# liwanyue123/SRBD-NMPC-Solver

Measured on AMD Instinct MI355X. Metric: SRBD OCP-QP solves/sec (N=20, nx=12, nu=12, fp64) at 1/2/4/8 MI355X, higher is better.
Workload: dtype f64

## Files before the change

srbd-nmpc-solver_amd/csrc/qp_group.h:

```cpp
#pragma once

#include <hip/hip_runtime.h>

#include <type_traits>
#include <utility>

namespace srbd {

constexpr int kMaxDim = 12;
constexpr int kGroup = 16;
constexpr int kVecLane = 15;

template <int I>
using ic = std::integral_constant<int, I>;

template <int B, int E, typename F>
__device__ __forceinline__ void sfor(F&& f) {
  if constexpr (B < E) {
    f(ic<B>{});
    sfor<B + 1, E>(static_cast<F&&>(f));
  }
}
template <int B, int E, typename F>
__device__ __forceinline__ void sfor_down(F&& f) {
  if constexpr (B < E) {
    f(ic<E - 1>{});
    sfor_down<B, E - 1>(static_cast<F&&>(f));
  }
}

template <int SRC>
__device__ __forceinline__ double bc(double v) {
  static_assert(SRC >= 0 && SRC < kGroup, "row_newbcast source lane");
  return __builtin_amdgcn_update_dpp(0.0, v, 0x150 + SRC, 0xf, 0xf, true);
}

template <int SRC>
__device__ __forceinline__ float bc(float v) {
  static_assert(SRC >= 0 && SRC < kGroup, "row_newbcast source lane");
  return __builtin_bit_cast(
      float, __builtin_amdgcn_update_dpp(0, __builtin_bit_cast(int, v), 0x150 + SRC, 0xf, 0xf, true));
}

__device__ __forceinline__ void lds_wave_fence() {
  asm volatile("" ::: "memory");
  __builtin_amdgcn_wave_barrier();
}

template <typename T>
__device__ __forceinline__ void opaque(T& x) {
  asm volatile("" : "+v"(x));
}
template <typename T, int... Is>
__device__ __forceinline__ void launder_impl(T (&v)[12], std::integer_sequence<int, Is...>) {
  (opaque(v[Is]), ...);
}
template <typename T>
__device__ __forceinline__ void launder(T (&v)[12]) {
  launder_impl(v, std::make_integer_sequence<int, 12>{});
}

#define SRBD_FMAC_DPP(D, S0, S1, LANE) "v_fmac_f64_dpp " D ", " S0 ", " S1 " row_newbcast:" #LANE " row_mask:0xf bank_mask:0xf\n\t"

template <int SRC>
__device__ __forceinline__ void fma_bcast_src(double (&C)[12], const double (&X)[12], double y) {
  static_assert(SRC >= 0 && SRC < kGroup, "row_newbcast source lane");
  asm volatile(
      "s_nop 1\n\t"
      "v_fmac_f64_dpp %0, %12, %24 row_newbcast:%25 row_mask:0xf bank_mask:0xf\n\t"
      "v_fmac_f64_dpp %1, %13, %24 row_newbcast:%25 row_mask:0xf bank_mask:0xf\n\t"
      "v_fmac_f64_dpp %2, %14, %24 row_newbcast:%25 row_mask:0xf bank_mask:0xf\n\t"
      "v_fmac_f64_dpp %3, %15, %24 row_newbcast:%25 row_mask:0xf bank_mask:0xf\n\t"
      "v_fmac_f64_dpp %4, %16, %24 row_newbcast:%25 row_mask:0xf bank_mask:0xf\n\t"
      "v_fmac_f64_dpp %5, %17, %24 row_newbcast:%25 row_mask:0xf bank_mask:0xf\n\t"
      "v_fmac_f64_dpp %6, %18, %24 row_newbcast:%25 row_mask:0xf bank_mask:0xf\n\t"
      "v_fmac_f64_dpp %7, %19, %24 row_newbcast:%25 row_mask:0xf bank_mask:0xf\n\t"
      "v_fmac_f64_dpp %8, %20, %24 row_newbcast:%25 row_mask:0xf bank_mask:0xf\n\t"
      "v_fmac_f64_dpp %9, %21, %24 row_newbcast:%25 row_mask:0xf bank_mask:0xf\n\t"
      "v_fmac_f64_dpp %10, %22, %24 row_newbcast:%25 row_mask:0xf bank_mask:0xf\n\t"
      "v_fmac_f64_dpp %11, %23, %24 row_newbcast:%25 row_mask:0xf bank_mask:0xf"
      : "+v"(C[0]), "+v"(C[1]), "+v"(C[2]), "+v"(C[3]), "+v"(C[4]), "+v"(C[5]), "+v"(C[6]),
        "+v"(C[7]), "+v"(C[8]), "+v"(C[9]), "+v"(C[10]), "+v"(C[11])
      : "v"(X[0]), "v"(X[1]), "v"(X[2]), "v"(X[3]), "v"(X[4]), "v"(X[5]), "v"(X[6]), "v"(X[7]),
        "v"(X[8]), "v"(X[9]), "v"(X[10]), "v"(X[11]), "v"(y), "i"(SRC));
}

__device__ __forceinline__ void fma_bcast_lanes(double (&C)[12], double x, double y) {
  asm volatile(
      "s_nop 1\n\t"
      "v_fmac_f64_dpp %0, %12, %13 row_newbcast:0 row_mask:0xf bank_mask:0xf\n\t"
      "v_fmac_f64_dpp %1, %12, %13 row_newbcast:1 row_mask:0xf bank_mask:0xf\n\t"
      "v_fmac_f64_dpp %2, %12, %13 row_newbcast:2 row_mask:0xf bank_mask:0xf\n\t"
      "v_fmac_f64_dpp %3, %12, %13 row_newbcast:3 row_mask:0xf bank_mask:0xf\n\t"
      "v_fmac_f64_dpp %4, %12, %13 row_newbcast:4 row_mask:0xf bank_mask:0xf\n\t"
      "v_fmac_f64_dpp %5, %12, %13 row_newbcast:5 row_mask:0xf bank_mask:0xf\n\t"
      "v_fmac_f64_dpp %6, %12, %13 row_newbcast:6 row_mask:0xf bank_mask:0xf\n\t"
      "v_fmac_f64_dpp %7, %12, %13 row_newbcast:7 row_mask:0xf bank_mask:0xf\n\t"
      "v_fmac_f64_dpp %8, %12, %13 row_newbcast:8 row_mask:0xf bank_mask:0xf\n\t"
      "v_fmac_f64_dpp %9, %12, %13 row_newbcast:9 row_mask:0xf bank_mask:0xf\n\t"
      "v_fmac_f64_dpp %10, %12, %13 row_newbcast:10 row_mask:0xf bank_mask:0xf\n\t"
      "v_fmac_f64_dpp %11, %12, %13 row_newbcast:11 row_mask:0xf bank_mask:0xf"
      : "+v"(C[0]), "+v"(C[1]), "+v"(C[2]), "+v"(C[3]), "+v"(C[4]), "+v"(C[5]), "+v"(C[6]),
        "+v"(C[7]), "+v"(C[8]), "+v"(C[9]), "+v"(C[10]), "+v"(C[11])
      : "v"(x), "v"(y));
}

template <int SRC>
__device__ __forceinline__ void fma_bcast_src(float (&C)[12], const float (&X)[12], float y) {
  static_assert(SRC >= 0 && SRC < kGroup, "row_newbcast source lane");
  asm volatile(
      "s_nop 1\n\t"
      "v_fmac_f32_dpp %0, %12, %24 row_newbcast:%25 row_mask:0xf bank_mask:0xf\n\t"
      "v_fmac_f32_dpp %1, %13, %24 row_newbcast:%25 row_mask:0xf bank_mask:0xf\n\t"
      "v_fmac_f32_dpp %2, %14, %24 row_newbcast:%25 row_mask:0xf bank_mask:0xf\n\t"
      "v_fmac_f32_dpp %3, %15, %24 row_newbcast:%25 row_mask:0xf bank_mask:0xf\n\t"
      "v_fmac_f32_dpp %4, %16, %24 row_newbcast:%25 row_mask:0xf bank_mask:0xf\n\t"
      "v_fmac_f32_dpp %5, %17, %24 row_newbcast:%25 row_mask:0xf bank_mask:0xf\n\t"
      "v_fmac_f32_dpp %6, %18, %24 row_newbcast:%25 row_mask:0xf bank_mask:0xf\n\t"
      "v_fmac_f32_dpp %7, %19, %24 row_newbcast:%25 row_mask:0xf bank_mask:0xf\n\t"
      "v_fmac_f32_dpp %8, %20, %24 row_newbcast:%25 row_mask:0xf bank_mask:0xf\n\t"
      "v_fmac_f32_dpp %9, %21, %24 row_newbcast:%25 row_mask:0xf bank_mask:0xf\n\t"
      "v_fmac_f32_dpp %10, %22, %24 row_newbcast:%25 row_mask:0xf bank_mask:0xf\n\t"
      "v_fmac_f32_dpp %11, %23, %24 row_newbcast:%25 row_mask:0xf bank_mask:0xf"
      : "+v"(C[0]), "+v"(C[1]), "+v"(C[2]), "+v"(C[3]), "+v"(C[4]), "+v"(C[5]), "+v"(C[6]),
        "+v"(C[7]), "+v"(C[8]), "+v"(C[9]), "+v"(C[10]), "+v"(C[11])
      : "v"(X[0]), "v"(X[1]), "v"(X[2]), "v"(X[3]), "v"(X[4]), "v"(X[5]), "v"(X[6]), "v"(X[7]),
        "v"(X[8]), "v"(X[9]), "v"(X[10]), "v"(X[11]), "v"(y), "i"(SRC));
}
__device__ __forceinline__ void fma_bcast_lanes(float (&C)[12], float x, float y) {
  asm volatile(
      "s_nop 1\n\t"
      "v_fmac_f32_dpp %0, %12, %13 row_newbcast:0 row_mask:0xf bank_mask:0xf\n\t"
      "v_fmac_f32_dpp %1, %12, %13 row_newbcast:1 row_mask:0xf bank_mask:0xf\n\t"
      "v_fmac_f32_dpp %2, %12, %13 row_newbcast:2 row_mask:0xf bank_mask:0xf\n\t"
      "v_fmac_f32_dpp %3, %12, %13 row_newbcast:3 row_mask:0xf bank_mask:0xf\n\t"
      "v_fmac_f32_dpp %4, %12, %13 row_newbcast:4 row_mask:0xf bank_mask:0xf\n\t"
      "v_fmac_f32_dpp %5, %12, %13 row_newbcast:5 row_mask:0xf bank_mask:0xf\n\t"
      "v_fmac_f32_dpp %6, %12, %13 row_newbcast:6 row_mask:0xf bank_mask:0xf\n\t"
      "v_fmac_f32_dpp %7, %12, %13 row_newbcast:7 row_mask:0xf bank_mask:0xf\n\t"
      "v_fmac_f32_dpp %8, %12, %13 row_newbcast:8 row_mask:0xf bank_mask:0xf\n\t"
      "v_fmac_f32_dpp %9, %12, %13 row_newbcast:9 row_mask:0xf bank_mask:0xf\n\t"
      "v_fmac_f32_dpp %10, %12, %13 row_newbcast:10 row_mask:0xf bank_mask:0xf\n\t"
      "v_fmac_f32_dpp %11, %12, %13 row_newbcast:11 row_mask:0xf bank_mask:0xf"
      : "+v"(C[0]), "+v"(C[1]), "+v"(C[2]), "+v"(C[3]), "+v"(C[4]), "+v"(C[5]), "+v"(C[6]),
        "+v"(C[7]), "+v"(C[8]), "+v"(C[9]), "+v"(C[10]), "+v"(C[11])
      : "v"(x), "v"(y));
}

__device__ __forceinline__ double dot_bcast(const double (&M)[12], double x, double acc) {
  asm volatile(
      "s_nop 1\n\t"
      "v_fmac_f64_dpp %0, %1, %2 row_newbcast:0 row_mask:0xf bank_mask:0xf\n\t"
      "v_fmac_f64_dpp %0, %1, %3 row_newbcast:1 row_mask:0xf bank_mask:0xf\n\t"
      "v_fmac_f64_dpp %0, %1, %4 row_newbcast:2 row_mask:0xf bank_mask:0xf\n\t"
      "v_fmac_f64_dpp %0, %1, %5 row_newbcast:3 row_mask:0xf bank_mask:0xf\n\t"
      "v_fmac_f64_dpp %0, %1, %6 row_newbcast:4 row_mask:0xf bank_mask:0xf\n\t"
      "v_fmac_f64_dpp %0, %1, %7 row_newbcast:5 row_mask:0xf bank_mask:0xf\n\t"
      "v_fmac_f64_dpp %0, %1, %8 row_newbcast:6 row_mask:0xf bank_mask:0xf\n\t"
      "v_fmac_f64_dpp %0, %1, %9 row_newbcast:7 row_mask:0xf bank_mask:0xf\n\t"
      "v_fmac_f64_dpp %0, %1, %10 row_newbcast:8 row_mask:0xf bank_mask:0xf\n\t"
      "v_fmac_f64_dpp %0, %1, %11 row_newbcast:9 row_mask:0xf bank_mask:0xf\n\t"
      "v_fmac_f64_dpp %0, %1, %12 row_newbcast:10 row_mask:0xf bank_mask:0xf\n\t"
      "v_fmac_f64_dpp %0, %1, %13 row_newbcast:11 row_mask:0xf bank_mask:0xf"
      : "+&v"(acc)
      : "v"(x), "v"(M[0]), "v"(M[1]), "v"(M[2]), "v"(M[3]), "v"(M[4]), "v"(M[5]), "v"(M[6]), "v"(M[7]), "v"(M[8]), "v"(M[9]), "v"(M[10]), "v"(M[11]));
  return acc;
}
__device__ __forceinline__ float dot_bcast(const float (&M)[12], float x, float acc) {
  asm volatile(
      "s_nop 1\n\t"
      "v_fmac_f32_dpp %0, %1, %2 row_newbcast:0 row_mask:0xf bank_mask:0xf\n\t"
      "v_fmac_f32_dpp %0, %1, %3 row_newbcast:1 row_mask:0xf bank_mask:0xf\n\t"
      "v_fmac_f32_dpp %0, %1, %4 row_newbcast:2 row_mask:0xf bank_mask:0xf\n\t"
      "v_fmac_f32_dpp %0, %1, %5 row_newbcast:3 row_mask:0xf bank_mask:0xf\n\t"
      "v_fmac_f32_dpp %0, %1, %6 row_newbcast:4 row_mask:0xf bank_mask:0xf\n\t"
      "v_fmac_f32_dpp %0, %1, %7 row_newbcast:5 row_mask:0xf bank_mask:0xf\n\t"
      "v_fmac_f32_dpp %0, %1, %8 row_newbcast:6 row_mask:0xf bank_mask:0xf\n\t"
      "v_fmac_f32_dpp %0, %1, %9 row_newbcast:7 row_mask:0xf bank_mask:0xf\n\t"
      "v_fmac_f32_dpp %0, %1, %10 row_newbcast:8 row_mask:0xf bank_mask:0xf\n\t"
      "v_fmac_f32_dpp %0, %1, %11 row_newbcast:9 row_mask:0xf bank_mask:0xf\n\t"
      "v_fmac_f32_dpp %0, %1, %12 row_newbcast:10 row_mask:0xf bank_mask:0xf\n\t"
      "v_fmac_f32_dpp %0, %1, %13 row_newbcast:11 row_mask:0xf bank_mask:0xf"
      : "+&v"(acc)
      : "v"(x), "v"(M[0]), "v"(M[1]), "v"(M[2]), "v"(M[3]), "v"(M[4]), "v"(M[5]), "v"(M[6]), "v"(M[7]), "v"(M[8]), "v"(M[9]), "v"(M[10]), "v"(M[11]));
  return acc;
}

__device__ __forceinline__ void dot_bcast2(const double (&M1)[12], const double (&M2)[12], double x,
                                           double& acc1, double& acc2) {
  asm volatile(
      "s_nop 1\n\t"
      "v_fmac_f64_dpp %0, %2, %3 row_newbcast:0 row_mask:0xf bank_mask:0xf\n\t"
      "v_fmac_f64_dpp %1, %2, %15 row_newbcast:0 row_mask:0xf bank_mask:0xf\n\t"
      "v_fmac_f64_dpp %0, %2, %4 row_newbcast:1 row_mask:0xf bank_mask:0xf\n\t"
      "v_fmac_f64_dpp %1, %2, %16 row_newbcast:1 row_mask:0xf bank_mask:0xf\n\t"
      "v_fmac_f64_dpp %0, %2, %5 row_newbcast:2 row_mask:0xf bank_mask:0xf\n\t"
      "v_fmac_f64_dpp %1, %2, %17 row_newbcast:2 row_mask:0xf bank_mask:0xf\n\t"
      "v_fmac_f64_dpp %0, %2, %6 row_newbcast:3 row_mask:0xf bank_mask:0xf\n\t"
      "v_fmac_f64_dpp %1, %2, %18 row_newbcast:3 row_mask:0xf bank_mask:0xf\n\t"
      "v_fmac_f64_dpp %0, %2, %7 row_newbcast:4 row_mask:0xf bank_mask:0xf\n\t"
      "v_fmac_f64_dpp %1, %2, %19 row_newbcast:4 row_mask:0xf bank_mask:0xf\n\t"
      "v_fmac_f64_dpp %0, %2, %8 row_newbcast:5 row_mask:0xf bank_mask:0xf\n\t"
      "v_fmac_f64_dpp %1, %2, %20 row_newbcast:5 row_mask:0xf bank_mask:0xf\n\t"
      "v_fmac_f64_dpp %0, %2, %9 row_newbcast:6 row_mask:0xf bank_mask:0xf\n\t"
      "v_fmac_f64_dpp %1, %2, %21 row_newbcast:6 row_mask:0xf bank_mask:0xf\n\t"
      "v_fmac_f64_dpp %0, %2, %10 row_newbcast:7 row_mask:0xf bank_mask:0xf\n\t"
      "v_fmac_f64_dpp %1, %2, %22 row_newbcast:7 row_mask:0xf bank_mask:0xf\n\t"
      "v_fmac_f64_dpp %0, %2, %11 row_newbcast:8 row_mask:0xf bank_mask:0xf\n\t"
      "v_fmac_f64_dpp %1, %2, %23 row_newbcast:8 row_mask:0xf bank_mask:0xf\n\t"
      "v_fmac_f64_dpp %0, %2, %12 row_newbcast:9 row_mask:0xf bank_mask:0xf\n\t"
      "v_fmac_f64_dpp %1, %2, %24 row_newbcast:9 row_mask:0xf bank_mask:0xf\n\t"
      "v_fmac_f64_dpp %0, %2, %13 row_newbcast:10 row_mask:0xf bank_mask:0xf\n\t"
      "v_fmac_f64_dpp %1, %2, %25 row_newbcast:10 row_mask:0xf bank_mask:0xf\n\t"
      "v_fmac_f64_dpp %0, %2, %14 row_newbcast:11 row_mask:0xf bank_mask:0xf\n\t"
      "v_fmac_f64_dpp %1, %2, %26 row_newbcast:11 row_mask:0xf bank_mask:0xf"
      : "+&v"(acc1), "+&v"(acc2)
      : "v"(x), "v"(M1[0]), "v"(M1[1]), "v"(M1[2]), "v"(M1[3]), "v"(M1[4]), "v"(M1[5]), "v"(M1[6]), "v"(M1[7]), "v"(M1[8]), "v"(M1[9]), "v"(M1[10]), "v"(M1[11]),
        "v"(M2[0]), "v"(M2[1]), "v"(M2[2]), "v"(M2[3]), "v"(M2[4]), "v"(M2[5]), "v"(M2[6]), "v"(M2[7]), "v"(M2[8]), "v"(M2[9]), "v"(M2[10]), "v"(M2[11]));
}
__device__ __forceinline__ void dot_bcast2(const float (&M1)[12], const float (&M2)[12], float x,
                                           float& acc1, float& acc2) {
  asm volatile(
      "s_nop 1\n\t"
      "v_fmac_f32_dpp %0, %2, %3 row_newbcast:0 row_mask:0xf bank_mask:0xf\n\t"
      "v_fmac_f32_dpp %1, %2, %15 row_newbcast:0 row_mask:0xf bank_mask:0xf\n\t"
      "v_fmac_f32_dpp %0, %2, %4 row_newbcast:1 row_mask:0xf bank_mask:0xf\n\t"
      "v_fmac_f32_dpp %1, %2, %16 row_newbcast:1 row_mask:0xf bank_mask:0xf\n\t"
      "v_fmac_f32_dpp %0, %2, %5 row_newbcast:2 row_mask:0xf bank_mask:0xf\n\t"
      "v_fmac_f32_dpp %1, %2, %17 row_newbcast:2 row_mask:0xf bank_mask:0xf\n\t"
      "v_fmac_f32_dpp %0, %2, %6 row_newbcast:3 row_mask:0xf bank_mask:0xf\n\t"
      "v_fmac_f32_dpp %1, %2, %18 row_newbcast:3 row_mask:0xf bank_mask:0xf\n\t"
      "v_fmac_f32_dpp %0, %2, %7 row_newbcast:4 row_mask:0xf bank_mask:0xf\n\t"
      "v_fmac_f32_dpp %1, %2, %19 row_newbcast:4 row_mask:0xf bank_mask:0xf\n\t"
      "v_fmac_f32_dpp %0, %2, %8 row_newbcast:5 row_mask:0xf bank_mask:0xf\n\t"
      "v_fmac_f32_dpp %1, %2, %20 row_newbcast:5 row_mask:0xf bank_mask:0xf\n\t"
      "v_fmac_f32_dpp %0, %2, %9 row_newbcast:6 row_mask:0xf bank_mask:0xf\n\t"
      "v_fmac_f32_dpp %1, %2, %21 row_newbcast:6 row_mask:0xf bank_mask:0xf\n\t"
      "v_fmac_f32_dpp %0, %2, %10 row_newbcast:7 row_mask:0xf bank_mask:0xf\n\t"
      "v_fmac_f32_dpp %1, %2, %22 row_newbcast:7 row_mask:0xf bank_mask:0xf\n\t"
      "v_fmac_f32_dpp %0, %2, %11 row_newbcast:8 row_mask:0xf bank_mask:0xf\n\t"
      "v_fmac_f32_dpp %1, %2, %23 row_newbcast:8 row_mask:0xf bank_mask:0xf\n\t"
      "v_fmac_f32_dpp %0, %2, %12 row_newbcast:9 row_mask:0xf bank_mask:0xf\n\t"
      "v_fmac_f32_dpp %1, %2, %24 row_newbcast:9 row_mask:0xf bank_mask:0xf\n\t"
      "v_fmac_f32_dpp %0, %2, %13 row_newbcast:10 row_mask:0xf bank_mask:0xf\n\t"
      "v_fmac_f32_dpp %1, %2, %25 row_newbcast:10 row_mask:0xf bank_mask:0xf\n\t"
      "v_fmac_f32_dpp %0, %2, %14 row_newbcast:11 row_mask:0xf bank_mask:0xf\n\t"
      "v_fmac_f32_dpp %1, %2, %26 row_newbcast:11 row_mask:0xf bank_mask:0xf"
      : "+&v"(acc1), "+&v"(acc2)
      : "v"(x), "v"(M1[0]), "v"(M1[1]), "v"(M1[2]), "v"(M1[3]), "v"(M1[4]), "v"(M1[5]), "v"(M1[6]), "v"(M1[7]), "v"(M1[8]), "v"(M1[9]), "v"(M1[10]), "v"(M1[11]),
        "v"(M2[0]), "v"(M2[1]), "v"(M2[2]), "v"(M2[3]), "v"(M2[4]), "v"(M2[5]), "v"(M2[6]), "v"(M2[7]), "v"(M2[8]), "v"(M2[9]), "v"(M2[10]), "v"(M2[11]));
}

template <typename T>
__device__ __forceinline__ T fmadd(T a, T b, T c) {
  return __builtin_fma(a, b, c);
}
template <>
__device__ __forceinline__ float fmadd<float>(float a, float b, float c) {
  return __builtin_fmaf(a, b, c);
}

__device__ __forceinline__ void load12(const double* __restrict__ p, double (&v)[12]) {
  const double2* p2 = reinterpret_cast<const double2*>(p);
  sfor<0, 6>([&](auto i) {
    constexpr int I = decltype(i)::value;
    double2 t = p2[I];
    v[2 * I] = t.x;
    v[2 * I + 1] = t.y;
  });
}
__device__ __forceinline__ void load12_nt(const double* __restrict__ p, double (&v)[12]) {
  typedef double dv2 __attribute__((ext_vector_type(2)));
  const dv2* p2 = reinterpret_cast<const dv2*>(p);
  sfor<0, 6>([&](auto i) {
    constexpr int I = decltype(i)::value;
    dv2 t = __builtin_nontemporal_load(p2 + I);
    v[2 * I] = t.x;
    v[2 * I + 1] = t.y;
  });
}
__device__ __forceinline__ void load12_nt(const float* __restrict__ p, float (&v)[12]) {
  typedef float fv2 __attribute__((ext_vector_type(2)));
  const fv2* p2 = reinterpret_cast<const fv2*>(p);
  sfor<0, 6>([&](auto i) {
    constexpr int I = decltype(i)::value;
    fv2 t = __builtin_nontemporal_load(p2 + I);
    v[2 * I] = t.x;
    v[2 * I + 1] = t.y;
  });
}
__device__ __forceinline__ void store12(double* __restrict__ p, const double (&v)[12]) {
  double2* p2 = reinterpret_cast<double2*>(p);
  sfor<0, 6>([&](auto i) {
    constexpr int I = decltype(i)::value;
    p2[I] = make_double2(v[2 * I], v[2 * I + 1]);
  });
}

__device__ __forceinline__ void load12(const float* __restrict__ p, float (&v)[12]) {
  const float2* p2 = reinterpret_cast<const float2*>(p);
  sfor<0, 6>([&](auto i) {
    constexpr int I = decltype(i)::value;
    float2 t = p2[I];
    v[2 * I] = t.x;
    v[2 * I + 1] = t.y;
  });
}
__device__ __forceinline__ void store12(float* __restrict__ p, const float (&v)[12]) {
  float2* p2 = reinterpret_cast<float2*>(p);
  sfor<0, 6>([&](auto i) {
    constexpr int I = decltype(i)::value;
    p2[I] = make_float2(v[2 * I], v[2 * I + 1]);
  });
}

template <typename T>
__device__ __forceinline__ void load_col_pad(const T* __restrict__ p, int rows, bool col_ok,
                                             T (&v)[12]) {
  sfor<0, 12>([&](auto i) {
    constexpr int I = decltype(i)::value;
    v[I] = (col_ok && I < rows) ? p[I] : T(0);
  });
}

__host__ __device__ constexpr int packed_col(int j) { return j * 12 - j * (j - 1) / 2; }

template <typename T>
__device__ __forceinline__ void store_packed_col(T* pk, int lane, const T (&v)[12]) {
  const int cj = packed_col(lane) - lane;
  sfor<0, 12>([&](auto i) {
    constexpr int I = decltype(i)::value;
    if (I >= lane) pk[cj + I] = v[I];
  });
}
template <typename Ptr, typename T>
__device__ __forceinline__ void load_packed_sym(Ptr pk, int r, T (&v)[12]) {
  const int cr = packed_col(r) - r;
  sfor<0, 12>([&](auto j) {
    constexpr int J = decltype(j)::value;
    v[J] = pk[J <= r ? packed_col(J) + r - J : cr + J];
  });
}
template <typename T>
__device__ __forceinline__ void load_packed_lrow_d(const T* pk, int r, T (&v)[12]) {
  sfor<0, 12>([&](auto j) {
    constexpr int J = decltype(j)::value;
    const T x = pk[packed_col(J) + r - J];
    v[J] = J <= r ? x : T(0);
  });
}
template <typename T>
__device__ __forceinline__ void load_packed_lcol_d(const T* pk, int c, T (&v)[12]) {
  const int cc = packed_col(c) - c;
  sfor<0, 12>([&](auto i) {
    constexpr int I = decltype(i)::value;
    const T x = pk[cc + I];
    v[I] = I >= c ? x : T(0);
  });
}
template <typename T>
__device__ __forceinline__ void load_packed_lrow(const T* pk, int r, T (&v)[12]) {
  sfor<0, 12>([&](auto j) {
    constexpr int J = decltype(j)::value;
    const T x = pk[packed_col(J) + r - J];
    v[J] = J < r ? x : T(0);
  });
}
template <typename T>
__device__ __forceinline__ void load_packed_lcol(const T* pk, int c, T (&v)[12]) {
  const int cc = packed_col(c) - c;
  sfor<0, 12>([&](auto i) {
    constexpr int I = decltype(i)::value;
    const T x = pk[cc + I];
    v[I] = I > c ? x : T(0);
  });
}

}
```

srbd-nmpc-solver_amd/csrc/riccati_unconstr_impl.h:

```cpp
namespace srbd {
namespace SRBD_NS {

using real = SRBD_REAL;


struct HbmSrc {
  const ProblemArgsT<real>& a;
  int qp;
  __device__ const real* at(const real* base, int nstage, int blk, int k) const {
    return a.layout == 1 ? base + ((size_t)k * a.batch + qp) * blk
                         : base + ((size_t)qp * nstage + k) * blk;
  }
  __device__ const real* A(int k) const { return at(a.A, a.N, 144, k); }
  __device__ const real* B(int k) const { return at(a.B, a.N, 144, k); }
  __device__ const real* b(int k) const { return at(a.b, a.N, 12, k); }
  __device__ const real* Q(int k) const { return at(a.Q, a.N + 1, 144, k); }
  __device__ const real* S(int k) const { return at(a.S, a.N, 144, k); }
  __device__ const real* R(int k) const { return at(a.R, a.N, 144, k); }
  __device__ const real* q(int k) const { return at(a.q, a.N + 1, 12, k); }
  __device__ const real* r(int k) const { return at(a.r, a.N, 12, k); }
  __device__ real* rec(int k) const { return a.ws + ((size_t)k * a.batch + qp) * kWsStage; }
  real* img = nullptr;
  int gq = 0;
  __device__ real* kept(int k) const { return img + (k * 4 + gq) * kWsStage; }
  template <class StoreRec>
  __device__ void store_stage(int k, StoreRec&& store) const;
};

template <class Src>
constexpr bool keeps_turnaround = std::is_same_v<Src, HbmSrc> && sizeof(real) == 8;

constexpr int kImgA = 0, kImgB = 144, kImgb = 288, kImgQ = 300, kImgS = 444, kImgR = 588,
              kImgq = 732, kImgr = 744, kImgStage = 756, kImgRec = kImgQ;
static_assert(kImgRec + kWsStage <= kImgStage, "a record fits its stage slot past A, B, b");

struct LdsSrc {
  real* img;
  real* grec = nullptr;
  int batch = 0, qp = 0;
  __device__ real* slot(int k) const { return img + k * kImgStage; }
  __device__ const real* A(int k) const { return slot(k) + kImgA; }
  __device__ const real* B(int k) const { return slot(k) + kImgB; }
  __device__ const real* b(int k) const { return slot(k) + kImgb; }
  __device__ const real* Q(int k) const { return slot(k) + kImgQ; }
  __device__ const real* S(int k) const { return slot(k) + kImgS; }
  __device__ const real* R(int k) const { return slot(k) + kImgR; }
  __device__ const real* q(int k) const { return slot(k) + kImgq; }
  __device__ const real* r(int k) const { return slot(k) + kImgr; }
  __device__ real* rec(int k) const {
    return grec ? grec + ((size_t)k * batch + qp) * kWsStage : slot(k) + kImgRec;
  }
};

__device__ __forceinline__ void store_rec_P(real* rec, int lane, const real (&P)[12]) {
  if (lane < kMaxDim) store_packed_col(rec + kWsP, lane, P);
  if (lane == kVecLane) store12(rec + kWsp, P);
}
__device__ __forceinline__ void store_rec(real* rec, int lane, const real (&Kc)[12], const real (&P)[12]) {
  const bool isv = lane == kVecLane;
  if (lane < kMaxDim || isv) {
    const int c = isv ? kMaxDim : lane;
    sfor<0, 12>([&](auto m) {
      constexpr int M = decltype(m)::value;
      rec[kWsK + M * kWsRow + c] = Kc[M];
    });
  }
  store_rec_P(rec, lane, P);
}

constexpr int kRecHotStages = 4;

template <class StoreRec>
__device__ void HbmSrc::store_stage(int k, StoreRec&& store) const {
  if (!img) {
    store(rec(k));
    return;
  }
  if (k < 2) {
    store(kept(k));
    lds_wave_fence();
    return;
  }
  store(img + gq * kWsStage);
  lds_wave_fence();
  const int qp0 = qp - gq;
  const int nq = a.batch - qp0 < 4 ? a.batch - qp0 : 4;
  constexpr int kPiecesPerRec = kWsStage * (int)sizeof(real) / 16;
  const int pieces = nq * kPiecesPerRec;
  typedef double d2 __attribute__((ext_vector_type(2)));
  const d2* src = reinterpret_cast<const d2*>(img);
  d2* dst = reinterpret_cast<d2*>(a.ws + ((size_t)k * a.batch + qp0) * kWsStage);
  const int l = (int)(threadIdx.x & 63);
  if (k >= kRecHotStages) {
    for (int p = l; p < pieces; p += 16 * nq) __builtin_nontemporal_store(src[p], &dst[p]);
  } else {
    for (int p = l; p < pieces; p += 16 * nq) dst[p] = src[p];
  }
  lds_wave_fence();
}

__device__ __forceinline__ void store_riccati_out(const ProblemArgsT<real>& a, int qp, int k, int lane,
                                                  const real (&F)[12], const real (&Kc)[12]) {
  const int N = a.N;
  const bool own = lane < kMaxDim, isv = lane == kVecLane;
  if (a.P && own) store12(a.P + ((size_t)qp * (N + 1) + k) * 144 + (size_t)lane * 12, F);
  if (a.p && isv) store12(a.p + ((size_t)qp * (N + 1) + k) * 12, F);
  if (k < N) {
    if (a.K && own) store12(a.K + ((size_t)qp * N + k) * 144 + (size_t)lane * 12, Kc);
    if (a.k && isv) store12(a.k + ((size_t)qp * N + k) * 12, Kc);
  }
}

template <class Src>
__device__ __forceinline__ void fwd_sweep(const ProblemArgsT<real>& a, const Src& src, const int qp,
                                          const int lane, real* so = nullptr) {
  constexpr int nx = 12, nu = 12;
  const int N = a.N;
  const bool own = lane < kMaxDim;
  const int row = own ? lane : kMaxDim - 1;
  real xv = own ? a.x0[(size_t)qp * nx + lane] : real(0.0);
  bool bad = false;
  real* xo = a.x + (size_t)qp * (N + 1) * nx;
  real* uo = a.u + (size_t)qp * N * nu;
  real* po = a.pi + (size_t)qp * (N + 1) * nx;
  real Pr[12], Kr[12], Ar[12], pv, kv, bv;
  auto load_rows = [&](int k, real (&P_)[12], real (&K_)[12], real (&A__)[12], real& p_, real& k_,
                       real& b_) {
    const real* rec = src.rec(k);
    load_packed_sym(rec + kWsP, row, P_);
    p_ = rec[kWsp + row];
    if (k < N) {
      const real* kr = rec + kWsK + row * kWsRow;
      const real* Ab = src.A(k);
      sfor<0, 12>([&](auto j) {
        constexpr int J = decltype(j)::value;
        K_[J] = kr[J];
        A__[J] = Ab[J * 12 + row];
      });
      k_ = kr[12];
      b_ = src.b(k)[row];
    }
  };
  auto load_rows_kept = [&](int k, real (&P_)[12], real (&K_)[12], real (&A__)[12], real& p_, real& k_,
                            real& b_) {
    if constexpr (keeps_turnaround<Src>) {
      const auto rec = (const __attribute__((address_space(3))) real*)src.kept(k);
      load_packed_sym(rec + kWsP, row, P_);
      p_ = rec[kWsp + row];
      const auto kr = rec + kWsK + row * kWsRow;
      const real* Ab = src.A(k);
      sfor<0, 12>([&](auto j) {
        constexpr int J = decltype(j)::value;
        K_[J] = kr[J];
        A__[J] = Ab[J * 12 + row];
      });
      k_ = kr[12];
      b_ = src.b(k)[row];
    }
  };
  auto kept = [&](int k) { return keeps_turnaround<Src> && k < 2 && k < N; };
  if (kept(0)) {
    load_rows_kept(0, Pr, Kr, Ar, pv, kv, bv);
  } else {
    load_rows(0, Pr, Kr, Ar, pv, kv, bv);
  }
#pragma unroll 1
  for (int k = 0; k <= N; ++k) {
    real Br[12];
    if (k < N) {
      const real* Bb = src.B(k);
      sfor<0, 12>([&](auto j) { Br[decltype(j)::value] = Bb[decltype(j)::value * 12 + row]; });
    }
    real Pn[12], Kn[12], An[12], pvn = real(0.0), kvn = real(0.0), bvn = real(0.0);
    if (k < N) {
      if (kept(k + 1)) {
        load_rows_kept(k + 1, Pn, Kn, An, pvn, kvn, bvn);
      } else {
        load_rows(k + 1, Pn, Kn, An, pvn, kvn, bvn);
      }
    }
    real bx[12];
    sfor<0, 12>([&](auto j) {
      constexpr int J = decltype(j)::value;
      bx[J] = bc<J>(xv);
    });
    real pp = pv;
    sfor<0, 12>([&](auto j) {
      constexpr int J = decltype(j)::value;
      pp = fmadd(Pr[J], bx[J], pp);
    });
    if (own) {
      xo[(size_t)k * nx + lane] = xv;
      po[(size_t)k * nx + lane] = pp;
      if (so) {
        so[k * nx + lane] = xv;
        so[(2 * N + 1) * nx + k * nx + lane] = pp;
      }
    }
    if (k == N) break;
    real uu = kv, xn = bv;
    sfor<0, 12>([&](auto j) {
      constexpr int J = decltype(j)::value;
      uu = fmadd(Kr[J], bx[J], uu);
      xn = fmadd(Ar[J], bx[J], xn);
    });
    if (own) {
      uo[(size_t)k * nu + lane] = uu;
      if (so) so[(N + 1) * nx + k * nu + lane] = uu;
    }
    xn = dot_bcast(Br, uu, xn);
    bad |= own && (!(uu == uu) || !(xn == xn));
    xv = xn;
    sfor<0, 12>([&](auto j) {
      constexpr int J = decltype(j)::value;
      Pr[J] = Pn[J];
      Kr[J] = Kn[J];
      Ar[J] = An[J];
    });
    pv = pvn;
    kv = kvn;
    bv = bvn;
  }
  if (a.status || a.iter) {
    const unsigned long long m = __ballot(bad);
    const int shift = (threadIdx.x & 63) & ~(kGroup - 1);
    const bool any_bad = ((m >> shift) & 0xffffull) != 0;
    if (lane == 0) {
      if (a.status) a.status[qp] = any_bad ? 3 : 0;
      if (a.iter) a.iter[qp] = 0;
    }
  }
}

template <bool SQRT, class Src>
__device__ __forceinline__ void solve_qp(const ProblemArgsT<real>& a, const Src& src, const int qp,
                                         const int lane, real* so = nullptr) {
  const int N = a.N;
  const bool isv = lane == kVecLane;
  const bool own = lane < kMaxDim;
  const int col = own ? lane : kMaxDim - 1;
  const real reg = a.reg;

  real P[12];
  if (isv) {
    load12(src.q(N), P);
  } else {
    load12(src.Q(N) + col * 12, P);
  }
  store_rec_P(src.rec(N), lane, P);
  store_riccati_out(a, qp, N, lane, P, P);
  if constexpr (SQRT) sqrt_factor(P, lane);

  real A_[12], B_[12];
#pragma unroll 1
  for (int k = N - 1; k >= 0; --k) {
    if (isv) {
      load12(src.b(k), A_);
      sfor<0, 12>([&](auto i) { B_[decltype(i)::value] = real(0.0); });
    } else {
      load12(src.A(k) + col * 12, A_);
      load12(src.B(k) + col * 12, B_);
    }
    auto loadR = [&](real (&Rc)[12]) {
      if (isv) {
        sfor<0, 12>([&](auto i) { Rc[decltype(i)::value] = real(0.0); });
      } else {
        load12(src.R(k) + col * 12, Rc);
      }
    };
    auto loadSQ = [&](real (&Sc)[12], real (&Qc)[12]) {
      if (isv) {
        load12(src.r(k), Sc);
        load12(src.q(k), Qc);
      } else {
        load12(src.S(k) + col * 12, Sc);
        load12(src.Q(k) + col * 12, Qc);
      }
    };
    StageFactor<real> f;
    tstamp(0);
    if constexpr (SQRT) {
      riccati_step_sqrt<1, false>(P, A_, B_, loadR, loadSQ, lane, reg, f);
    } else {
      riccati_step<1, false>(P, A_, B_, loadR, loadSQ, lane, reg, f);
    }
    if constexpr (std::is_same_v<Src, HbmSrc>) {
      src.store_stage(k, [&](real* r) { store_rec(r, lane, f.Kc, f.F); });
    } else {
      store_rec(src.rec(k), lane, f.Kc, f.F);
    }
    tstamp(11);
    store_riccati_out(a, qp, k, lane, f.F, f.Kc);
    sfor<0, 12>([&](auto i) {
      constexpr int I = decltype(i)::value;
      P[I] = f.F[I];
    });
    if constexpr (SQRT) sqrt_factor(P, lane);
  }
  tstamp(12);
  fwd_sweep(a, src, qp, lane, so);
  tstamp(13);
}

template <bool SQRT>
__global__ void __launch_bounds__(256, 2) riccati_unconstr_kernel(ProblemArgsT<real> a) {
  const int gid = blockIdx.x * blockDim.x + threadIdx.x;
  const int qp = gid >> 4;
  if (qp >= a.batch) return;
  if constexpr (sizeof(real) == 8) {
    __shared__ __attribute__((aligned(16))) real rec_img[4 * 2 * 4 * kWsStage];
    static_assert(sizeof(rec_img) <= 64 * 1024, "static LDS limit");
    HbmSrc src{a, qp};
    src.gq = (threadIdx.x >> 4) & 3;
    src.img = rec_img + (threadIdx.x >> 6) * 2 * 4 * kWsStage;
    solve_qp<SQRT>(a, src, qp, threadIdx.x & (kGroup - 1));
  } else {
    solve_qp<SQRT>(a, HbmSrc{a, qp}, qp, threadIdx.x & (kGroup - 1));
  }
}

constexpr int kRealsPerDma = 16 / (int)sizeof(real);
constexpr int kLdsCopyThreads = 512;

__device__ __forceinline__ const real* img_source(const ProblemArgsT<real>& a, int qp, int e) {
  const int N = a.N;
  const int k = e / kImgStage, o = e - k * kImgStage;
  const size_t s = (size_t)qp * N + k, s1 = (size_t)qp * (N + 1) + k;
  if (o >= kImgQ && o < kImgS) return a.Q + s1 * 144 + (o - kImgQ);
  if (o >= kImgq && o < kImgr) return a.q + s1 * 12 + (o - kImgq);
  if (k >= N) return nullptr;
  if (o < kImgB) return a.A + s * 144 + o;
  if (o < kImgb) return a.B + s * 144 + (o - kImgB);
  if (o < kImgQ) return a.b + s * 12 + (o - kImgb);
  if (o < kImgR) return a.S + s * 144 + (o - kImgS);
  if (o < kImgq) return a.R + s * 144 + (o - kImgR);
  return a.r + s * 12 + (o - kImgr);
}

__device__ __forceinline__ void lds_copy_range(const ProblemArgsT<real>& a, real* img, int qp, int e0, int e1,
                                               int t, int nthr) {
  const int wave_off = (t >> 6) * 64 * kRealsPerDma;
  for (int c0 = e0; c0 < e1; c0 += nthr * kRealsPerDma) {
    const int e = c0 + t * kRealsPerDma;
    const real* g = e < e1 ? img_source(a, qp, e) : nullptr;
    if (g)
      __builtin_amdgcn_global_load_lds((const __attribute__((address_space(1))) void*)g,
                                       (__attribute__((address_space(3))) void*)(img + c0 + wave_off), 16,
                                       0, 0);
  }
}
__device__ __forceinline__ void lds_copy_qp(const ProblemArgsT<real>& a, real* img, int qp) {
  lds_copy_range(a, img, qp, 0, (a.N + 1) * kImgStage, threadIdx.x, kLdsCopyThreads);
  tstamp(14);
  asm volatile("s_waitcnt vmcnt(0)" ::: "memory");
  __syncthreads();
  tstamp(15);
}

template <bool SQRT>
__global__ void __launch_bounds__(kLdsCopyThreads, 1) riccati_unconstr_lds_kernel(ProblemArgsT<real> a) {
  extern __shared__ __attribute__((aligned(16))) unsigned char lds_raw[];
  real* img = reinterpret_cast<real*>(lds_raw);
  const int qp = blockIdx.x;
  tstamp(16);
  lds_copy_qp(a, img, qp);
  if (threadIdx.x >= kGroup) return;
  solve_qp<SQRT>(a, LdsSrc{img}, qp, threadIdx.x);
}

size_t lds_image_bytes(int N) { return (size_t)(N + 1) * kImgStage * sizeof(real); }
size_t lds_res_bytes(int N) { return lds_image_bytes(N) + (size_t)(3 * N + 2) * 12 * sizeof(real); }


constexpr int kResThreads = 256;
constexpr int kResStages = kResThreads / 12;
constexpr int kResWavesMax = 8;

__device__ __forceinline__ void max_nan(real& m, real v) {
  v = v < real(0) ? -v : v;
  if (v > m || v != v) m = v;
}

struct ResGlobal {
  const ProblemArgsT<real>& a;
  int qp;
  __device__ const real* at(const real* base, int nstage, size_t blk, int k) const {
    return a.layout == 1 ? base + ((size_t)k * a.batch + qp) * blk : base + ((size_t)qp * nstage + k) * blk;
  }
  __device__ const real* A(int k) const { return at(a.A, a.N, (size_t)a.nx * a.nx, k); }
  __device__ const real* B(int k) const { return at(a.B, a.N, (size_t)a.nx * a.nu, k); }
  __device__ const real* b(int k) const { return at(a.b, a.N, a.nx, k); }
  __device__ const real* Q(int k) const { return at(a.Q, a.N + 1, (size_t)a.nx * a.nx, k); }
  __device__ const real* S(int k) const { return at(a.S, a.N, (size_t)a.nx * a.nu, k); }
  __device__ const real* R(int k) const { return at(a.R, a.N, (size_t)a.nu * a.nu, k); }
  __device__ const real* q(int k) const { return at(a.q, a.N + 1, a.nx, k); }
  __device__ const real* r(int k) const { return at(a.r, a.N, a.nu, k); }
  __device__ const real* x() const { return a.x + (size_t)qp * (a.N + 1) * a.nx; }
  __device__ const real* u() const { return a.u + (size_t)qp * a.N * a.nu; }
  __device__ const real* pi() const { return a.pi + (size_t)qp * (a.N + 1) * a.nx; }
};
struct ResLds : LdsSrc {
  const real* so;
  int N;
  __device__ const real* x() const { return so; }
  __device__ const real* u() const { return so + (N + 1) * 12; }
  __device__ const real* pi() const { return so + (2 * N + 1) * 12; }
};

template <class Acc, int DIM = 0>
__device__ __forceinline__ void unconstr_residuals_body(const ProblemArgsT<real>& a, const Acc& acc, int qp, int t) {
  const int N = a.N, nx = DIM ? DIM : a.nx, nu = DIM ? DIM : a.nu;
  if (a.stat) {
    real* tab = a.stat + (size_t)qp * a.stat_rows * kStatCols;
    for (int i = t; i < a.stat_rows * kStatCols; i += blockDim.x) tab[i] = real(0);
  }
  const real* x = acc.x();
  const real* u = acc.u();
  const real* pi = acc.pi();
  const int i = t % 12;
  real mg = real(0), mb = real(0), ob = real(0);
  for (int k = t / 12; t < kResStages * 12 && k <= N; k += kResStages) {
    const real* xk = x + (size_t)k * nx;
    if (k < N) {
      const real* uk = u + (size_t)k * nu;
      const real* xn = x + (size_t)(k + 1) * nx;
      const real* pn = pi + (size_t)(k + 1) * nx;
      const real* A = acc.A(k);
      const real* B = acc.B(k);
      if (i < nu) {
        const real* S = acc.S(k);
        const real* R = acc.R(k);
        const real* r = acc.r(k);
        real ru = real(0), sx = real(0), bp = real(0);
        for (int j = 0; j < nu; ++j) ru += R[(size_t)j * nu + i] * uk[j];
        for (int j = 0; j < nx; ++j) sx += S[(size_t)j * nu + i] * xk[j];
        for (int j = 0; j < nx; ++j) bp += B[(size_t)i * nx + j] * pn[j];
        max_nan(mg, ru + sx + r[i] + bp);
        ob += uk[i] * (real(0.5) * ru + r[i] + sx);
      }
      if (i < nx) {
        const real* b = acc.b(k);
        real v = b[i] - xn[i];
        for (int j = 0; j < nx; ++j) v += A[(size_t)j * nx + i] * xk[j];
        for (int j = 0; j < nu; ++j) v += B[(size_t)j * nx + i] * uk[j];
        max_nan(mb, v);
      }
    }
    if (k > 0 && i < nx) {
      const real* Q = acc.Q(k);
      const real* q = acc.q(k);
      real qx = real(0), g = q[i] - pi[(size_t)k * nx + i];
      for (int j = 0; j < nx; ++j) qx += Q[(size_t)j * nx + i] * xk[j];
      g += qx;
      if (k < N) {
        const real* uk = u + (size_t)k * nu;
        const real* pn = pi + (size_t)(k + 1) * nx;
        const real* A = acc.A(k);
        const real* S = acc.S(k);
        for (int j = 0; j < nu; ++j) g += S[(size_t)i * nu + j] * uk[j];
        for (int j = 0; j < nx; ++j) g += A[(size_t)i * nx + j] * pn[j];
      }
      max_nan(mg, g);
      ob += xk[i] * (real(0.5) * qx + q[i]);
    }
  }
  for (int m = 32; m >= 1; m >>= 1) {
    const real og = __shfl_xor(mg, m), obb = __shfl_xor(mb, m);
    if (og > mg || og != og) mg = og;
    if (obb > mb || obb != obb) mb = obb;
    ob += __shfl_xor(ob, m);
  }
  __shared__ real part[3][kResWavesMax];
  const int w = t / 64;
  if ((t & 63) == 0) {
    part[0][w] = mg;
    part[1][w] = mb;
    part[2][w] = ob;
  }
  __syncthreads();
  if (t == 0) {
    mg = part[0][0], mb = part[1][0], ob = part[2][0];
    for (int j = 1; j < kResThreads / 64; ++j) {
      if (part[0][j] > mg || part[0][j] != part[0][j]) mg = part[0][j];
      if (part[1][j] > mb || part[1][j] != part[1][j]) mb = part[1][j];
      ob += part[2][j];
    }
    if (a.res) {
      a.res[(size_t)qp * 4 + 0] = mg;
      a.res[(size_t)qp * 4 + 1] = mb;
      a.res[(size_t)qp * 4 + 2] = real(0);
      a.res[(size_t)qp * 4 + 3] = real(0);
    }
    if (a.obj) a.obj[qp] = ob;
    if (a.stat) {
      real* row = a.stat + (size_t)qp * a.stat_rows * kStatCols;
      row[6] = mg;
      row[7] = mb;
      row[10] = ob;
    }
    if (a.status && (mg != mg || mb != mb)) a.status[qp] = 3;
  }
}

__global__ void __launch_bounds__(kResThreads) unconstr_residuals_kernel(ProblemArgsT<real> a) {
  unconstr_residuals_body(a, ResGlobal{a, (int)blockIdx.x}, (int)blockIdx.x, (int)threadIdx.x);
}

template <bool SQRT>
__global__ void __launch_bounds__(kLdsCopyThreads, 1) riccati_unconstr_lds_res_kernel(ProblemArgsT<real> a) {
  extern __shared__ __attribute__((aligned(16))) unsigned char lds_raw[];
  real* img = reinterpret_cast<real*>(lds_raw);
  real* so = img + (a.N + 1) * kImgStage;
  const int qp = blockIdx.x;
  tstamp(16);
  lds_copy_qp(a, img, qp);
  LdsSrc src{img};
  src.grec = a.ws;
  src.batch = a.batch;
  src.qp = qp;
  if (threadIdx.x < kGroup) solve_qp<SQRT>(a, src, qp, threadIdx.x, so);
  __syncthreads();
  ResLds acc{};
  acc.img = img;
  acc.so = so;
  acc.N = a.N;
  unconstr_residuals_body(a, acc, qp, (int)threadIdx.x);
}

template <bool FULL>
__global__ void __launch_bounds__(256) unconstr_residuals_group_kernel(ProblemArgsT<real> a) {
  __shared__ __attribute__((aligned(16))) real tb_all[(256 / kGroup) * 144];
  const int qp = (int)((blockIdx.x * blockDim.x + threadIdx.x) >> 4);
  const int lane = threadIdx.x & (kGroup - 1);
  if (qp >= a.batch) return;
  real* const tb = tb_all + (threadIdx.x >> 4) * 144;
  const int N = a.N, nx = FULL ? 12 : a.nx, nu = FULL ? 12 : a.nu;
  if (a.stat) {
    real* tab = a.stat + (size_t)qp * a.stat_rows * kStatCols;
    for (int i = lane; i < a.stat_rows * kStatCols; i += kGroup) tab[i] = real(0);
  }
  const bool smaj = a.layout == 1;
  auto at = [&](const real* base, int nstage, size_t blk, int k) -> const real* {
    return smaj ? base + ((size_t)k * a.batch + qp) * blk : base + ((size_t)qp * nstage + k) * blk;
  };
  const size_t nxx = (size_t)nx * nx, nxu = (size_t)nx * nu, nuu = (size_t)nu * nu;
  const real* x = a.x + (size_t)qp * (N + 1) * nx;
  const real* u = a.u + (size_t)qp * N * nu;
  const real* pi = a.pi + (size_t)qp * (N + 1) * nx;
  const int li = lane < kMaxDim ? lane : 0;
  const bool xl = lane < nx, ul = lane < nu;
  auto colv = [&](const real* blk, int rows, int cols, real (&v)[12]) {
    if constexpr (FULL) {
      load12(blk + li * 12, v);
    } else {
      load_col_pad(blk + (size_t)li * rows, rows, lane < cols, v);
    }
  };
  auto row_sum = [&](const real (&T)[12]) -> real {
    lds_wave_fence();
    if (lane < kMaxDim) store12(tb + lane * 12, T);
    lds_wave_fence();
    real s = real(0);
    sfor<0, 12>([&](auto j) { s += tb[decltype(j)::value * 12 + li]; });
    return s;
  };
  real mg = real(0), mb = real(0), ob = real(0);
#pragma unroll 1
  for (int k = 0; k <= N; ++k) {
    const real xk = xl ? x[(size_t)k * nx + lane] : real(0);
    real T[12];
    real gx = real(0);
    if (k > 0) {
      real Qc[12];
      colv(at(a.Q, N + 1, nxx, k), nx, nx, Qc);
      sfor<0, 12>([&](auto i) { T[decltype(i)::value] = Qc[decltype(i)::value] * xk; });
      const real qx = row_sum(T);
      const real qk = xl ? at(a.q, N + 1, nx, k)[lane] : real(0);
      gx = qx + qk - (xl ? pi[(size_t)k * nx + lane] : real(0));
      if (xl) ob += xk * (real(0.5) * qx + qk);
    }
    if (k < N) {
      const real uk = ul ? u[(size_t)k * nu + lane] : real(0);
      const real xn = xl ? x[(size_t)(k + 1) * nx + lane] : real(0);
      const real pin = xl ? pi[(size_t)(k + 1) * nx + lane] : real(0);
      real Ac[12], Bc[12];
      colv(at(a.A, N, nxx, k), nx, nx, Ac);
      colv(at(a.B, N, nxu, k), nx, nu, Bc);
      const real atp = dot_bcast(Ac, pin, real(0));
      const real btp = dot_bcast(Bc, pin, real(0));
      sfor<0, 12>([&](auto i) {
        constexpr int I = decltype(i)::value;
        T[I] = fmadd(Ac[I], xk, Bc[I] * uk);
      });
      const real axbu = row_sum(T);
      if (xl) max_nan(mb, axbu + at(a.b, N, nx, k)[lane] - xn);
      real Sc[12], Rc[12];
      colv(at(a.S, N, nxu, k), nu, nx, Sc);
      colv(at(a.R, N, nuu, k), nu, nu, Rc);
      const real stu = dot_bcast(Sc, uk, real(0));
      sfor<0, 12>([&](auto i) {
        constexpr int I = decltype(i)::value;
        T[I] = fmadd(Rc[I], uk, Sc[I] * xk);
      });
      const real rusx = row_sum(T);
      const real rk = ul ? at(a.r, N, nu, k)[lane] : real(0);
      if (ul) {
        max_nan(mg, rusx + rk + btp);
        ob += uk * (real(0.5) * rusx + rk);
      }
      if (xl) ob += real(0.5) * xk * stu;
      gx += stu + atp;
    }
    if (k > 0 && xl) max_nan(mg, gx);
  }
  sfor<0, 4>([&](auto s) {
    constexpr int M = 8 >> decltype(s)::value;
    const real og = __shfl_xor(mg, M, kGroup), obb = __shfl_xor(mb, M, kGroup);
    if (og > mg || og != og) mg = og;
    if (obb > mb || obb != obb) mb = obb;
    ob += __shfl_xor(ob, M, kGroup);
  });
  if (lane == 0) {
    if (a.res) {
      a.res[(size_t)qp * 4 + 0] = mg;
      a.res[(size_t)qp * 4 + 1] = mb;
      a.res[(size_t)qp * 4 + 2] = real(0);
      a.res[(size_t)qp * 4 + 3] = real(0);
    }
    if (a.obj) a.obj[qp] = ob;
    if (a.stat) {
      real* row = a.stat + (size_t)qp * a.stat_rows * kStatCols;
      row[6] = mg;
      row[7] = mb;
      row[10] = ob;
    }
    if (a.status && (mg != mg || mb != mb)) a.status[qp] = 3;
  }
}

constexpr int kResGroupMin = 256;

hipError_t launch_residuals(const ProblemArgsT<real>& a, hipStream_t stream) {
  if (a.batch <= 0) return hipSuccess;
  if (a.batch <= kResGroupMin) {
    hipLaunchKernelGGL(unconstr_residuals_kernel, dim3((unsigned)a.batch), dim3(kResThreads), 0, stream, a);
    return hipGetLastError();
  }
  const unsigned blocks = (unsigned)(((long long)a.batch * kGroup + 255) / 256);
  if (a.nx == 12 && a.nu == 12) {
    hipLaunchKernelGGL(unconstr_residuals_group_kernel<true>, dim3(blocks), dim3(256), 0, stream, a);
  } else {
    hipLaunchKernelGGL(unconstr_residuals_group_kernel<false>, dim3(blocks), dim3(256), 0, stream, a);
  }
  return hipGetLastError();
}

constexpr int kLdsBatchMax = 256;
constexpr size_t kLdsBytesMax = 160 * 1024;
constexpr size_t kLdsResStatic = 1024;

bool use_lds_kernel(const ProblemArgsT<real>& a) {
  return a.layout == 0 && a.batch <= kLdsBatchMax && lds_image_bytes(a.N) <= kLdsBytesMax;
}

#if SRBD_WITH_LATENCY
#include "riccati_latency_impl.h"
bool lat_eligible(const ProblemArgsT<real>& a) { return use_lds_kernel(a) && lat_fits(a.N); }
#else
bool lat_eligible(const ProblemArgsT<real>&) { return false; }
#endif

bool fused_residuals(const ProblemArgsT<real>& a) {
  return a.fuse_res && (a.res || a.obj || a.stat) && a.nx == 12 && a.nu == 12 && use_lds_kernel(a) &&
         lds_res_bytes(a.N) + kLdsResStatic <= kLdsBytesMax;
}
bool reads_once(const ProblemArgsT<real>& a) {
  return a.nx == 12 && a.nu == 12 && use_lds_kernel(a) &&
         (fused_residuals(a) || !(a.res || a.obj || a.stat));
}

template <bool SQRT>
static hipError_t launch_alg(const ProblemArgsT<real>& a, hipStream_t stream) {
#if SRBD_WITH_LATENCY
  if (!SQRT && lat_eligible(a)) {
    if (fused_residuals(a)) {
      hipLaunchKernelGGL(riccati_latency_kernel<true>, dim3((unsigned)a.batch), dim3(kLatThreads),
                         lat_lds_bytes(a.N), stream, a);
    } else {
      hipLaunchKernelGGL(riccati_latency_kernel<false>, dim3((unsigned)a.batch), dim3(kLatThreads),
                         lat_lds_bytes(a.N), stream, a);
    }
    return hipGetLastError();
  }
#endif
  if (fused_residuals(a)) {
    hipLaunchKernelGGL(riccati_unconstr_lds_res_kernel<SQRT>, dim3((unsigned)a.batch), dim3(kLdsCopyThreads),
                       lds_res_bytes(a.N), stream, a);
    return hipGetLastError();
  }
  if (use_lds_kernel(a)) {
    const size_t bytes = lds_image_bytes(a.N);
    hipLaunchKernelGGL(riccati_unconstr_lds_kernel<SQRT>, dim3((unsigned)a.batch), dim3(kLdsCopyThreads), bytes,
                       stream, a);
    return hipGetLastError();
  }
  const int threads = 256;
  const long long lanes = (long long)a.batch * kGroup;
  const int blocks = (int)((lanes + threads - 1) / threads);
  hipLaunchKernelGGL(riccati_unconstr_kernel<SQRT>, dim3(blocks), dim3(threads), 0, stream, a);
  return hipGetLastError();
}

#if SRBD_WITH_LATENCY
bool server_ok(const ProblemArgsT<real>& a) {
  return a.batch == 1 && !a.ric_alg && lat_eligible(a) && reads_once(a);
}
hipError_t launch_server(const ProblemArgsT<real>& a, LatMailbox* mb, int epoch, int last_done,
                         long long idle_ticks, long long life_ticks, hipStream_t stream) {
  if (!server_ok(a)) return hipErrorInvalidValue;
  if (fused_residuals(a))
    hipLaunchKernelGGL(riccati_latency_server_kernel<true>, dim3(1), dim3(kLatThreads), lat_lds_bytes(a.N), stream,
                       a, mb, epoch, last_done, idle_ticks, life_ticks);
  else
    hipLaunchKernelGGL(riccati_latency_server_kernel<false>, dim3(1), dim3(kLatThreads), lat_lds_bytes(a.N), stream,
                       a, mb, epoch, last_done, idle_ticks, life_ticks);
  return hipGetLastError();
}
#endif

hipError_t prepare_device() {
  hipError_t e = hipFuncSetAttribute(reinterpret_cast<const void*>(&riccati_unconstr_lds_kernel<false>),
                                     hipFuncAttributeMaxDynamicSharedMemorySize, (int)kLdsBytesMax);
  if (e == hipSuccess)
    e = hipFuncSetAttribute(reinterpret_cast<const void*>(&riccati_unconstr_lds_kernel<true>),
                            hipFuncAttributeMaxDynamicSharedMemorySize, (int)kLdsBytesMax);
  if (e == hipSuccess)
    e = hipFuncSetAttribute(reinterpret_cast<const void*>(&riccati_unconstr_lds_res_kernel<false>),
                            hipFuncAttributeMaxDynamicSharedMemorySize, (int)(kLdsBytesMax - kLdsResStatic));
  if (e == hipSuccess)
    e = hipFuncSetAttribute(reinterpret_cast<const void*>(&riccati_unconstr_lds_res_kernel<true>),
                            hipFuncAttributeMaxDynamicSharedMemorySize, (int)(kLdsBytesMax - kLdsResStatic));
#if SRBD_WITH_LATENCY
  if (e == hipSuccess)
    e = hipFuncSetAttribute(reinterpret_cast<const void*>(&riccati_latency_kernel<false>),
                            hipFuncAttributeMaxDynamicSharedMemorySize, (int)(kLdsBytesMax - kLdsResStatic));
  if (e == hipSuccess)
    e = hipFuncSetAttribute(reinterpret_cast<const void*>(&riccati_latency_kernel<true>),
                            hipFuncAttributeMaxDynamicSharedMemorySize, (int)(kLdsBytesMax - kLdsResStatic));
  if (e == hipSuccess)
    e = hipFuncSetAttribute(reinterpret_cast<const void*>(&riccati_latency_server_kernel<false>),
                            hipFuncAttributeMaxDynamicSharedMemorySize, (int)(kLdsBytesMax - kLdsResStatic));
  if (e == hipSuccess)
    e = hipFuncSetAttribute(reinterpret_cast<const void*>(&riccati_latency_server_kernel<true>),
                            hipFuncAttributeMaxDynamicSharedMemorySize, (int)(kLdsBytesMax - kLdsResStatic));
#endif
  return e;
}

hipError_t launch(const ProblemArgsT<real>& a, hipStream_t stream) {
  if (a.batch <= 0) return hipSuccess;
  if (a.nx != 12 || a.nu != 12) return hipErrorInvalidValue;
  return a.ric_alg ? launch_alg<true>(a, stream) : launch_alg<false>(a, stream);
}

}
}
```

Measured before the change: 23.78 million.

## Keep stage-0 gain and cost-to-go in registers and fuse the first forward step

The backward Riccati sweep now keeps the final stage's K and P in registers. A new stage0_forward routine computes u0, pi0 and x1 directly from those registers, so stage 0 is no longer written to and read back from the LDS record image. The LDS keep slots shift to stages 1 and 2, and the forward sweep starts at stage 1 with x1 and the bad flag passed in. This trades extra live registers (24 doubles) and a special-case code path for fewer LDS round trips around the turnaround between sweeps.

```diff
diff --git a/srbd-nmpc-solver_amd/csrc/qp_group.h b/srbd-nmpc-solver_amd/csrc/qp_group.h
--- a/srbd-nmpc-solver_amd/csrc/qp_group.h
+++ b/srbd-nmpc-solver_amd/csrc/qp_group.h
@@ -145,6 +145,21 @@
       : "+v"(C[0]), "+v"(C[1]), "+v"(C[2]), "+v"(C[3]), "+v"(C[4]), "+v"(C[5]), "+v"(C[6]),
         "+v"(C[7]), "+v"(C[8]), "+v"(C[9]), "+v"(C[10]), "+v"(C[11])
       : "v"(x), "v"(y));
+}
+
+template <int SRC>
+__device__ __forceinline__ void fma_bcast_one(double& c, double x, double y) {
+  static_assert(SRC >= 0 && SRC < kGroup, "row_newbcast source lane");
+  asm volatile("s_nop 1\n\tv_fmac_f64_dpp %0, %1, %2 row_newbcast:%3 row_mask:0xf bank_mask:0xf"
+               : "+v"(c)
+               : "v"(x), "v"(y), "i"(SRC));
+}
+template <int SRC>
+__device__ __forceinline__ void fma_bcast_one(float& c, float x, float y) {
+  static_assert(SRC >= 0 && SRC < kGroup, "row_newbcast source lane");
+  asm volatile("s_nop 1\n\tv_fmac_f32_dpp %0, %1, %2 row_newbcast:%3 row_mask:0xf bank_mask:0xf"
+               : "+v"(c)
+               : "v"(x), "v"(y), "i"(SRC));
 }
 
 __device__ __forceinline__ double dot_bcast(const double (&M)[12], double x, double acc) {
diff --git a/srbd-nmpc-solver_amd/csrc/riccati_unconstr_impl.h b/srbd-nmpc-solver_amd/csrc/riccati_unconstr_impl.h
--- a/srbd-nmpc-solver_amd/csrc/riccati_unconstr_impl.h
+++ b/srbd-nmpc-solver_amd/csrc/riccati_unconstr_impl.h
@@ -22,7 +22,7 @@
   __device__ real* rec(int k) const { return a.ws + ((size_t)k * a.batch + qp) * kWsStage; }
   real* img = nullptr;
   int gq = 0;
-  __device__ real* kept(int k) const { return img + (k * 4 + gq) * kWsStage; }
+  __device__ real* kept(int k) const { return img + ((k - 1) * 4 + gq) * kWsStage; }
   template <class StoreRec>
   __device__ void store_stage(int k, StoreRec&& store) const;
 };
@@ -76,7 +76,8 @@
     store(rec(k));
     return;
   }
-  if (k < 2) {
+  if (k == 0) return;
+  if (k <= 2) {
     store(kept(k));
     lds_wave_fence();
     return;
@@ -113,13 +114,21 @@
 
 template <class Src>
 __device__ __forceinline__ void fwd_sweep(const ProblemArgsT<real>& a, const Src& src, const int qp,
-                                          const int lane, real* so = nullptr) {
+                                          const int lane, real* so = nullptr, const real x1 = real(0.0),
+                                          const bool bad0 = false) {
   constexpr int nx = 12, nu = 12;
+  constexpr int k0 = keeps_turnaround<Src> ? 1 : 0;
   const int N = a.N;
   const bool own = lane < kMaxDim;
   const int row = own ? lane : kMaxDim - 1;
-  real xv = own ? a.x0[(size_t)qp * nx + lane] : real(0.0);
+  real xv;
   bool bad = false;
+  if constexpr (keeps_turnaround<Src>) {
+    xv = x1;
+    bad = bad0;
+  } else {
+    xv = own ? a.x0[(size_t)qp * nx + lane] : real(0.0);
+  }
   real* xo = a.x + (size_t)qp * (N + 1) * nx;
   real* uo = a.u + (size_t)qp * N * nu;
   real* po = a.pi + (size_t)qp * (N + 1) * nx;
@@ -158,14 +167,14 @@
       b_ = src.b(k)[row];
     }
   };
-  auto kept = [&](int k) { return keeps_turnaround<Src> && k < 2 && k < N; };
-  if (kept(0)) {
-    load_rows_kept(0, Pr, Kr, Ar, pv, kv, bv);
+  auto kept = [&](int k) { return keeps_turnaround<Src> && k >= 1 && k <= 2 && k < N; };
+  if (kept(k0)) {
+    load_rows_kept(k0, Pr, Kr, Ar, pv, kv, bv);
   } else {
-    load_rows(0, Pr, Kr, Ar, pv, kv, bv);
+    load_rows(k0, Pr, Kr, Ar, pv, kv, bv);
   }
 #pragma unroll 1
-  for (int k = 0; k <= N; ++k) {
+  for (int k = k0; k <= N; ++k) {
     real Br[12];
     if (k < N) {
       const real* Bb = src.B(k);
@@ -232,6 +241,80 @@
   }
 }
 
+template <class Src>
+__device__ __forceinline__ bool stage0_forward(const ProblemArgsT<real>& a, const Src& src, const int qp,
+                                               const int lane, const real (&Kc)[12], const real (&F)[12],
+                                               real& x1) {
+  constexpr int nx = 12, nu = 12;
+  const bool own = lane < kMaxDim, isv = lane == kVecLane;
+  const int col = own ? lane : kMaxDim - 1;
+  const real xv = own ? a.x0[(size_t)qp * nx + lane] : real(0.0);
+  real M[12];
+  if (isv) {
+    load12(src.b(0), M);
+  } else {
+    load12(src.A(0) + col * 12, M);
+  }
+  real bx[12];
+  sfor<0, 12>([&](auto j) {
+    constexpr int J = decltype(j)::value;
+    bx[J] = bc<J>(xv);
+  });
+  int ln = lane;
+  opaque(ln);
+  auto mine = [&](const real (&v)[12]) {
+    real r = real(0.0);
+    sfor<0, 12>([&](auto i) {
+      constexpr int I = decltype(i)::value;
+      r = ln == I ? v[I] : r;
+    });
+    return r;
+  };
+  real acc[12];
+  sfor<0, 12>([&](auto i) { acc[decltype(i)::value] = bc<kVecLane>(Kc[decltype(i)::value]); });
+  sfor<0, 12>([&](auto j) {
+    constexpr int J = decltype(j)::value;
+    fma_bcast_src<J>(acc, Kc, bx[J]);
+  });
+  const real uu = mine(acc);
+  SRBD_PHASE_FENCE();
+  sfor<0, 12>([&](auto i) { acc[decltype(i)::value] = bc<kVecLane>(F[decltype(i)::value]); });
+  sfor<0, 12>([&](auto j) {
+    constexpr int J = decltype(j)::value;
+    sfor<0, 12>([&](auto i) {
+      constexpr int I = decltype(i)::value;
+      if constexpr (J <= I) {
+        fma_bcast_one<J>(acc[I], F[I], bx[J]);
+      } else {
+        fma_bcast_one<I>(acc[I], F[J], bx[J]);
+      }
+    });
+  });
+  const real pp = mine(acc);
+  SRBD_PHASE_FENCE();
+  sfor<0, 12>([&](auto i) { acc[decltype(i)::value] = bc<kVecLane>(M[decltype(i)::value]); });
+  sfor<0, 12>([&](auto j) {
+    constexpr int J = decltype(j)::value;
+    fma_bcast_src<J>(acc, M, bx[J]);
+  });
+  load12(src.B(0) + col * 12, M);
+  sfor<0, 12>([&](auto j) {
+    constexpr int J = decltype(j)::value;
+    bx[J] = bc<J>(uu);
+  });
+  sfor<0, 12>([&](auto j) {
+    constexpr int J = decltype(j)::value;
+    fma_bcast_src<J>(acc, M, bx[J]);
+  });
+  x1 = mine(acc);
+  if (own) {
+    a.x[(size_t)qp * (a.N + 1) * nx + lane] = xv;
+    a.pi[(size_t)qp * (a.N + 1) * nx + lane] = pp;
+    a.u[(size_t)qp * a.N * nu + lane] = uu;
+  }
+  return own && (!(uu == uu) || !(x1 == x1));
+}
+
 template <bool SQRT, class Src>
 __device__ __forceinline__ void solve_qp(const ProblemArgsT<real>& a, const Src& src, const int qp,
                                          const int lane, real* so = nullptr) {
@@ -252,6 +335,7 @@
   if constexpr (SQRT) sqrt_factor(P, lane);
 
   real A_[12], B_[12];
+  real K0[12] = {}, P0[12] = {};
 #pragma unroll 1
   for (int k = N - 1; k >= 0; --k) {
     if (isv) {
@@ -294,11 +378,21 @@
     sfor<0, 12>([&](auto i) {
       constexpr int I = decltype(i)::value;
       P[I] = f.F[I];
+      if constexpr (keeps_turnaround<Src>) {
+        K0[I] = f.Kc[I];
+        P0[I] = f.F[I];
+      }
     });
     if constexpr (SQRT) sqrt_factor(P, lane);
   }
   tstamp(12);
-  fwd_sweep(a, src, qp, lane, so);
+  if constexpr (keeps_turnaround<Src>) {
+    real x1;
+    const bool bad0 = stage0_forward(a, src, qp, lane, K0, P0, x1);
+    fwd_sweep(a, src, qp, lane, so, x1, bad0);
+  } else {
+    fwd_sweep(a, src, qp, lane, so);
+  }
   tstamp(13);
 }
 
```

Result: no change. 23.57 million (median of 2 runs) (-0.9%).
